# SciML/NeuralPDE.jl

Measured on NVIDIA H100. Metric: collocation-points/sec (loss+grad), higher is better.
Workload: dtype f32

## Files before the change

neuralpde.jl_b200/csrc/tc_common.cuh:

```cuda
#pragma once
#include <cuda_runtime.h>
#include <stdint.h>
#include "tc_types.h"
#include "ffma_kernel.cuh"
#include "tc_prims.cuh"
#include "tail.cuh"

namespace pinn {

constexpr int kNH = kTcThreads / 128;
static_assert(kTcThreads == 512, "the MMA chains are spread over four warpgroups");
constexpr int GW = 4;
constexpr int GWB = 2;

template <int N>
__device__ __forceinline__ float pick(const float* v, int idx) {
  float r = v[0];
#pragma unroll
  for (int i = 1; i < N; ++i) r = (idx == i) ? v[i] : r;
  return r;
}
template <int N>
__device__ __forceinline__ void add_at(float* v, int idx, float x) {
#pragma unroll
// ... 425 lines not shown
      const int n_params = P.n_params;
      for (int j = 0; j < n_params; ++j) {
        float v = warp_sum<float>(pbar[j] * g);
        if (lane == 0) atomicAdd(&partial[P.param_off + j], v);
      }
    }
  }
  __syncthreads();
}

struct DbgSpan {
  long long c0;
  unsigned long long g0;
};
__device__ __forceinline__ DbgSpan dbg_span_begin(const long long* dbg) {
  DbgSpan s{0, 0};
#ifdef PINN_DEBUG
  if (dbg && threadIdx.x == 0) {
    s.c0 = clock64();
    asm volatile("mov.u64 %0, %globaltimer;" : "=l"(s.g0));
  }
#endif
  return s;
}

template <typename CS>
__device__ __forceinline__ void cta_finish(const TcCommonArgs& a, const CS& cs, const DbgSpan& span, const Misc& ms,
                                           const DevProblem& P, bool want_grad) {
  extern __shared__ __align__(1024) uint8_t smem[];
  const int tid = threadIdx.x;
#ifdef PINN_DEBUG
  if (tid == 0 && cs.dbg) cs.dbg[999] = cs.dbg_n;
  if (a.dbg && tid == 0 && blockIdx.x < 250) {
    unsigned long long g1;
    unsigned int smid;
    asm volatile("mov.u64 %0, %globaltimer;" : "=l"(g1));
    asm volatile("mov.u32 %0, %smid;" : "=r"(smid));
    long long* rec = a.dbg + 1000 + 4 * blockIdx.x;
    rec[0] = (long long)span.g0; rec[1] = (long long)g1; rec[2] = clock64() - span.c0; rec[3] = smid;
  }
#endif
  if (tid < PINN_MAX_TERMS) a.term_sums[(long long)blockIdx.x * PINN_MAX_TERMS + tid] = ms.tsum[tid];
  if (a.tail.state)
    fused_tail<float, kTcThreads>(a.tail, a.partial, a.partial_stride, a.term_sums, P.n_theta, P.n_terms, want_grad ? 1 : 0,
                                  reinterpret_cast<float*>(smem + a.off_P));
}


template <int C, typename CS>
__device__ __forceinline__ void finish_forward(CS* cs, const DevTerm& tm, int slot, const Misc& ms, const float* bl, const Tid& t,
                                               const float (&u)[C]) {
  __syncthreads();
  dbg_mark(cs, 15);
#pragma unroll
  for (int c = 0; c < C; ++c) atomicAdd(&ms.scratch[c * kTcPts + t.p], u[c]);
  __syncthreads();
  if (t.hh == 0) {
    float s[C];
#pragma unroll
    for (int c = 0; c < C; ++c) s[c] = ms.scratch[c * kTcPts + t.p];
    s[0] += *bl;
    const int n_taps = tm.n_taps;
    for (int tt = 0; tt < n_taps; ++tt)
      if (tm.tap_slot[tt] == slot) {
        const int tch = tm.tap_ch[tt];
        float v = s[0];
#pragma unroll
        for (int c = 1; c < C; ++c) v = (tch == c) ? s[c] : v;
        ms.taps[tt * kTcPts + t.p] = v;
      }
  }
  __syncthreads();
  dbg_mark(cs, 16);
}

template <int C>
__device__ __forceinline__ void gather_ubar(const DevTerm& tm, int slot, const Misc& ms, int p, float (&ub)[C]) {
#pragma unroll
  for (int c = 0; c < C; ++c) ub[c] = 0.f;
  const int n_taps = tm.n_taps;
  for (int tt = 0; tt < n_taps; ++tt)
    if (tm.tap_slot[tt] == slot) {
      const float g = ms.tapbar[tt * kTcPts + p];
      const int tch = tm.tap_ch[tt];
#pragma unroll
      for (int c = 0; c < C; ++c) ub[c] += (tch == c) ? g : 0.f;
    }
}

template <int C>
__device__ __forceinline__ void last_layer_grad(const Tid& t, const float (&ub)[C], int nL, float* gw, float* gb, uint32_t u_tile,
                                                uint32_t h_tile, uint32_t h_stride, uint32_t h_lbo, uint32_t acol, int rows) {
  if (t.hh == 0) {
    const float s = warp_sum<float>(ub[0]);
    if (t.lane == 0) atomicAdd(gb, s);
    uint32_t w[8];
#pragma unroll
    for (int c = 0; c < 8; ++c) w[c] = 0u;
#pragma unroll
    for (int c = 0; c < C; ++c) {
      const uint32_t hi = tc::pack_bf16(ub[c], 0.f);
      w[c] = hi | (bf16x2_lo(ub[c], 0.f, hi) << 16);
    }
    sts_v4(u_tile + tc::swz_chunk(t.p, 0), w[0], w[1], w[2], w[3]);
    sts_v4(u_tile + tc::swz_chunk(t.p, 1), w[4], w[5], w[6], w[7]);
  }
  tc::fence_async_smem();
  __syncthreads();
  {
    const uint32_t idesc = tc::make_idesc(16, 1, 1);
    const uint64_t db = tc::make_desc(u_tile, 0, 1024);
#pragma unroll 1
    for (int c = 0; c < C; ++c)
      mma_chain(acol + 16 * c, tc::make_desc(h_tile + c * h_stride, h_lbo, 1024), db, 2048, 2048, kTcPts / 16, idesc, 0);
  }
  __syncthreads();
  if (t.hh == 0 && t.q * 32 < rows) {
    const int o = t.q * 32 + t.lane;
    float acc = 0.f;
#pragma unroll
    for (int c = 0; c < C; ++c) {
      float v[2];
      acc_ld2(t.lane_addr + acol + 16 * c + 2 * c, v);
      acc += v[0] + v[1];
    }
    if (o < nL) atomicAdd(gw + o, acc);
  }
  __syncthreads();
}

__device__ __forceinline__ void flush_wgrad(const Tid& t, uint32_t wcol, uint32_t bcol, int rows, int n_in, int n_out, float* gw,
                                            float* gb) {
  if (t.q * 32 < rows) {
    const int o = t.q * 32 + t.lane;
    if (t.hh == 0) {
      float v[2];
      acc_ld2(t.lane_addr + bcol, v);
      if (o < n_out) atomicAdd(gb + o, v[0]);
    }
    const int part = n_in / kNH;
#pragma unroll 1
    for (int k0 = t.hh * part; k0 < (t.hh + 1) * part; k0 += 4) {
      float v[4];
      acc_ld4(t.lane_addr + wcol + k0, v);
      if (o < n_out) {
#pragma unroll
        for (int i = 0; i < 4; ++i) atomicAdd(gw + o + (long long)n_out * (k0 + i), v[i]);
      }
    }
  }
}

template <int N1>
__device__ __forceinline__ void coord_tiles(const Tid& t, uint32_t b_tile, const float (&x)[PINN_MAX_IN],
                                            const int (&dir1)[N1 > 0 ? N1 : 1], bool x_lo) {
  if (t.tid >= kTcPts) return;
  uint32_t hi[4], lo[4];
#pragma unroll
  for (int k = 0; k < 4; ++k) {
    hi[k] = tc::pack_bf16(x[2 * k], x[2 * k + 1]);
    lo[k] = bf16x2_lo(x[2 * k], x[2 * k + 1], hi[k]);
  }
  const uint32_t c0a = b_tile + tc::swz_chunk(t.p, 0), c1a = b_tile + tc::swz_chunk(t.p, 1);
  sts_v4(c0a, hi[0], hi[1], hi[2], hi[3]);
  sts_v4(c1a, 0x00003f80u, 0u, 0u, 0u);
  if (x_lo) {
    sts_v4(c0a + (1 + N1) * kTileBytes, lo[0], lo[1], lo[2], lo[3]);
    sts_v4(c1a + (1 + N1) * kTileBytes, 0u, 0u, 0u, 0u);
  }
#pragma unroll
  for (int j = 0; j < N1; ++j) {
    const int d = dir1[j];
    uint32_t w[4];
#pragma unroll
    for (int k = 0; k < 4; ++k) w[k] = (d == 2 * k) ? 0x00003f80u : ((d == 2 * k + 1) ? 0x3f800000u : 0u);
    sts_v4(c0a + (1 + j) * kTileBytes, w[0], w[1], w[2], w[3]);
    sts_v4(c1a + (1 + j) * kTileBytes, 0u, 0u, 0u, 0u);
  }
}
template <int N1>
__device__ __forceinline__ void layer0_grad(const Tid& t, uint32_t z_tile, uint32_t z_stride, uint32_t z_lbo, uint32_t b_tile,
                                            bool x_lo, uint32_t acol, int rows, int n1w, int d_in, float* gw0, float* gb0) {
  tc::fence_async_smem();
  __syncthreads();
  {
    const uint32_t idesc = tc::make_idesc(16, 1, 1);
    const uint64_t a0 = tc::make_desc(z_tile, z_lbo, 1024);
    mma_chain(acol, a0, tc::make_desc(b_tile, 0, 1024), 2048, 2048, kTcPts / 16, idesc, 0);
    if (x_lo) mma_chain(acol, a0, tc::make_desc(b_tile + (1 + N1) * kTileBytes, 0, 1024), 2048, 2048, kTcPts / 16, idesc, 1);
#pragma unroll 1
    for (int j = 0; j < N1; ++j)
      mma_chain(acol, tc::make_desc(z_tile + (1 + j) * z_stride, z_lbo, 1024), tc::make_desc(b_tile + (1 + j) * kTileBytes, 0, 1024),
                2048, 2048, kTcPts / 16, idesc, 1);
  }
  __syncthreads();
  if (t.hh == 0 && t.q * 32 < rows) {
    const int o = t.q * 32 + t.lane;
    float v[16];
    tc::acc_ld16(t.lane_addr + acol, v);
    if (o < n1w) {
#pragma unroll
      for (int k = 0; k < PINN_MAX_IN; ++k)
        if (k < d_in) atomicAdd(gw0 + o + (long long)n1w * k, v[k]);
      atomicAdd(gb0 + o, v[8]);
    }
  }
}

#define PINN_TC_CASE(maxc, a1, a2, pu, CALL)                                                  \
  {                                                                                           \
    constexpr int A1 = a1, A2 = a2;                                                           \
    constexpr bool PU = pu;                                                                   \
    if constexpr (1 + A1 + A2 <= (maxc)) {                                                    \
      if (_ak == 1) { constexpr int AK = 1; CALL; } else { constexpr int AK = 0; CALL; }     \
    }                                                                                         \
  }                                                                                           \
  break
#define PINN_TC_DISPATCH(maxc, n1, n2, pure, ak, CALL)                                        \
  do {                                                                                        \
    const int _ak = (ak);                                                                     \
    const int _key = ((n1) * 8 + (n2)) * 2 + ((pure) ? 1 : 0);                                \
    switch (_key) {                                                                           \
      case (0 * 8 + 0) * 2: case (0 * 8 + 0) * 2 + 1: PINN_TC_CASE(maxc, 0, 0, true, CALL);   \
      case (1 * 8 + 0) * 2: case (1 * 8 + 0) * 2 + 1: PINN_TC_CASE(maxc, 1, 0, true, CALL);   \
      case (2 * 8 + 0) * 2: case (2 * 8 + 0) * 2 + 1: PINN_TC_CASE(maxc, 2, 0, true, CALL);   \
      case (3 * 8 + 0) * 2: case (3 * 8 + 0) * 2 + 1: PINN_TC_CASE(maxc, 3, 0, true, CALL);   \
      case (4 * 8 + 0) * 2: case (4 * 8 + 0) * 2 + 1: PINN_TC_CASE(maxc, 4, 0, true, CALL);   \
      case (1 * 8 + 1) * 2: case (1 * 8 + 1) * 2 + 1: PINN_TC_CASE(maxc, 1, 1, true, CALL);   \
      case (2 * 8 + 1) * 2 + 1: PINN_TC_CASE(maxc, 2, 1, true, CALL);                         \
      case (2 * 8 + 1) * 2: PINN_TC_CASE(maxc, 2, 1, false, CALL);                            \
      case (3 * 8 + 1) * 2 + 1: PINN_TC_CASE(maxc, 3, 1, true, CALL);                         \
      case (3 * 8 + 1) * 2: PINN_TC_CASE(maxc, 3, 1, false, CALL);                            \
      case (2 * 8 + 2) * 2 + 1: PINN_TC_CASE(maxc, 2, 2, true, CALL);                         \
      case (2 * 8 + 2) * 2: PINN_TC_CASE(maxc, 2, 2, false, CALL);                            \
      default: break;                                                                         \
    }                                                                                         \
  } while (0)

}
```

neuralpde.jl_b200/csrc/tc_kernel.cu:

```cuda
#include "tc_common.cuh"

namespace pinn {

using Fp = FpBlock<kTcW>;

struct CtaShared : CtaBase {
  int split, off_Q;
  uint8_t* stash;
  TcNetSmem nets[PINN_MAX_NETS];
};

struct LoopCtx {
  uint32_t fp;
  uint32_t bt;
  uint32_t tP;
  uint32_t tQ;
  float* gb;
  float* gw;
  uint32_t taddr;
  int act, split, p, lane, g0, g1, flag;
  __device__ __forceinline__ LoopCtx(uint32_t fp_, uint32_t bt_, uint32_t tP_, uint32_t tQ_, const Tid& t, int act_, int ng,
                                     int flag_, int split_ = 0, float* gb_ = nullptr, float* gw_ = nullptr)
      : fp(fp_), bt(bt_), tP(tP_), tQ(tQ_), gb(gb_), gw(gw_), taddr(t.lane_addr), act(act_), split(split_), p(t.p), lane(t.lane),
        g0(t.hh * (ng / kNH)), g1((t.hh + 1) * (ng / kNH)), flag(flag_) {}
};

template <int N1, int N2, bool PURE, int AK>
__device__ __forceinline__ void l0_fwd_loop(const LoopCtx lc, const PassInfo<N1, N2> pi, const float* xp, float* up) {
  constexpr int C = 1 + N1 + N2;
  float x[PINN_MAX_IN], u[C];
#pragma unroll
  for (int k = 0; k < PINN_MAX_IN; ++k) x[k] = xp[k];
#pragma unroll
  for (int c = 0; c < C; ++c) u[c] = up[c];
#pragma unroll 1
  for (int g = lc.g0; g < lc.g1; ++g) {
    float h[C][GW];
#pragma unroll
    for (int i = 0; i < GW; i += 2) {
      float za[C], zb2[C];
      first_layer_elem<kTcW>(lc.fp, pi, x, g * GW + i, za);
      first_layer_elem<kTcW>(lc.fp, pi, x, g * GW + i + 1, zb2);
      P2 zz[C], hv[C];
#pragma unroll
      for (int c = 0; c < C; ++c) zz[c] = mk2(za[c], zb2[c]);
      chain_fwd<N1, N2, PURE, AK, P2>(lc.act, pi.ch, zz, hv);
#pragma unroll
      for (int c = 0; c < C; ++c) { h[c][i] = hv[c].v.x; h[c][i + 1] = hv[c].v.y; }
      if (lc.flag) {
        const float w0 = lds_f32(lc.fp + (Fp::WL + g * GW + i) * 4), w1 = lds_f32(lc.fp + (Fp::WL + g * GW + i + 1) * 4);
#pragma unroll
        for (int c = 0; c < C; ++c) u[c] = fmaf(w1, hv[c].v.y, fmaf(w0, hv[c].v.x, u[c]));
      }
    }
#pragma unroll
    for (int c = 0; c < C; ++c) store_half(lc.tP + c * kTileBytes, lc.tQ + c * kTileBytes, lc.p, g * GW, h[c], lc.split != 0);
  }
#pragma unroll
  for (int c = 0; c < C; ++c) up[c] = u[c];
}

template <int C, int NK, bool SPLIT>
__device__ __forceinline__ void fwd_mma(float (&d)[C][16], uint32_t sP, uint32_t sQ, uint32_t whi, uint32_t wlo) {
  const int wg = threadIdx.x >> 7;
  const uint32_t aoff = (wg & 1) * 8192u, boff = (wg >> 1) * 32u * 128u;
  const uint64_t dwhi = tc::make_desc(whi + boff, 0, 1024), dwlo = tc::make_desc(wlo + boff, 0, 1024);
  tc::wgmma_fence();
#pragma unroll
  for (int c = 0; c < C; ++c) {
    const uint64_t dahi = tc::make_desc(sP + c * kTileBytes + aoff, 0, 1024);
    const uint64_t dalo = tc::make_desc(sQ + c * kTileBytes + aoff, 0, 1024);
#pragma unroll
    for (int pr = 0; pr < (SPLIT ? 3 : 1); ++pr) {
      const uint64_t a = (pr == 2) ? dalo : dahi, b = (pr == 1) ? dwlo : dwhi;
#pragma unroll
      for (int k = 0; k < NK; ++k)
        tc::wgmma_n32<0, 0>(d[c], a + 2 * k, b + 2 * k, (pr | k) ? 1u : 0u);
    }
  }
  tc::wgmma_commit();
  tc::wgmma_wait0();
}
template <int C>
__device__ __forceinline__ void fwd_mma_any(float (&d)[C][16], uint32_t sP, uint32_t sQ, uint32_t whi, uint32_t wlo, int nk,
                                            bool split) {
  switch (nk * 2 + (split ? 1 : 0)) {
    case 2: fwd_mma<C, 1, false>(d, sP, sQ, whi, wlo); break;
    case 3: fwd_mma<C, 1, true>(d, sP, sQ, whi, wlo); break;
    case 4: fwd_mma<C, 2, false>(d, sP, sQ, whi, wlo); break;
    case 5: fwd_mma<C, 2, true>(d, sP, sQ, whi, wlo); break;
    case 6: fwd_mma<C, 3, false>(d, sP, sQ, whi, wlo); break;
    case 7: fwd_mma<C, 3, true>(d, sP, sQ, whi, wlo); break;
    case 8: fwd_mma<C, 4, false>(d, sP, sQ, whi, wlo); break;
    default: fwd_mma<C, 4, true>(d, sP, sQ, whi, wlo); break;
  }
}

template <int N1, int N2, bool PURE, int AK, int C>
__device__ __forceinline__ void tl_fwd_frag(const float (&d)[C][16], const LoopCtx lc, const Chan<N1, N2> ch, float* scratch) {
  const int wg = threadIdx.x >> 7, w = (threadIdx.x >> 5) & 3;
  const int row0 = 64 * (wg & 1) + 16 * w + (lc.lane >> 2);
  const int col0 = 32 * (wg >> 1) + 2 * (lc.lane & 3);
  float u[2][C];
#pragma unroll
  for (int r = 0; r < 2; ++r)
#pragma unroll
    for (int c = 0; c < C; ++c) u[r][c] = 0.f;
#pragma unroll
  for (int i = 0; i < 16; i += 2) {
    const int rh = (i >> 1) & 1;
    const int row = row0 + 8 * rh, col = col0 + 8 * (i >> 2);
    P2 zz[C], hv[C];
    zz[0] = mk2(d[0][i] + lds_f32(lc.bt + col * 4), d[0][i + 1] + lds_f32(lc.bt + (col + 1) * 4));
#pragma unroll
    for (int c = 1; c < C; ++c) zz[c] = mk2(d[c][i], d[c][i + 1]);
    chain_fwd<N1, N2, PURE, AK, P2>(lc.act, ch, zz, hv);
    const uint32_t off = tc::swz_off(row, col);
#pragma unroll
    for (int c = 0; c < C; ++c) {
      const uint32_t hx = tc::pack_bf16(hv[c].v.x, hv[c].v.y);
      asm volatile("st.shared.b32 [%0], %1;" ::"r"(lc.tP + c * kTileBytes + off), "r"(hx) : "memory");
      if (lc.split)
        asm volatile("st.shared.b32 [%0], %1;" ::"r"(lc.tQ + c * kTileBytes + off), "r"(bf16x2_lo(hv[c].v.x, hv[c].v.y, hx))
                     : "memory");
    }
    if (lc.flag) {
      const float w0 = lds_f32(lc.fp + (Fp::WL + col) * 4), w1 = lds_f32(lc.fp + (Fp::WL + col + 1) * 4);
#pragma unroll
      for (int c = 0; c < C; ++c) u[rh][c] = fmaf(w1, hv[c].v.y, fmaf(w0, hv[c].v.x, u[rh][c]));
    }
  }
  if (lc.flag) {
#pragma unroll
    for (int r = 0; r < 2; ++r)
#pragma unroll
      for (int c = 0; c < C; ++c) {
        float s = u[r][c];
        s += __shfl_xor_sync(0xffffffffu, s, 1);
        s += __shfl_xor_sync(0xffffffffu, s, 2);
        if ((lc.lane & 3) == 0) atomicAdd(&scratch[c * kTcPts + row0 + 8 * r], s);
      }
  }
}

constexpr uint32_t kHalfBytes = kTileBytes / 2;

template <int C, int NK>
__device__ __forceinline__ void rec_mma(float (&d)[C][8], uint32_t sQ, uint32_t whi) {
  const uint64_t dw = tc::make_desc(whi + (threadIdx.x >> 7) * 16u * 128u, 0, 1024);
  tc::wgmma_fence();
#pragma unroll
  for (int c = 0; c < C; ++c) {
    const uint64_t da = tc::make_desc(sQ + c * kTileBytes, 0, 1024);
#pragma unroll
    for (int k = 0; k < NK; ++k) tc::wgmma_n16<0, 0>(d[c], da + 2 * k, dw + 2 * k, k ? 1u : 0u);
  }
  tc::wgmma_commit();
  tc::wgmma_wait0();
}
template <int C>
__device__ __forceinline__ void rec_mma_any(float (&d)[C][8], uint32_t sQ, uint32_t whi, int nk) {
  switch (nk) {
    case 1: rec_mma<C, 1>(d, sQ, whi); break;
    case 2: rec_mma<C, 2>(d, sQ, whi); break;
    case 3: rec_mma<C, 3>(d, sQ, whi); break;
    default: rec_mma<C, 4>(d, sQ, whi); break;
  }
}
template <int C, int NKO>
__device__ __forceinline__ void dgrad_mma(float (&d)[C][8], uint32_t sQ, uint32_t whi) {
  const uint32_t poff = kHalfBytes + (threadIdx.x >> 7) * 16u * 128u;
  const uint64_t dw = tc::make_desc(whi, 0, 1024);
  tc::wgmma_fence();
#pragma unroll
  for (int c = 0; c < C; ++c) {
    const uint64_t dz = tc::make_desc(sQ + c * kTileBytes + poff, 0, 1024);
#pragma unroll
    for (int k = 0; k < NKO; ++k)
      tc::wgmma_n16<1, 0>(d[c], dw + 128 * k, dz + 2 * k, k ? 1u : 0u);
  }
  tc::wgmma_commit();
  tc::wgmma_wait0();
}
template <int C>
__device__ __forceinline__ void dgrad_mma_any(float (&d)[C][8], uint32_t sQ, uint32_t whi, int nko) {
  switch (nko) {
    case 1: dgrad_mma<C, 1>(d, sQ, whi); break;
    case 2: dgrad_mma<C, 2>(d, sQ, whi); break;
    case 3: dgrad_mma<C, 3>(d, sQ, whi); break;
    default: dgrad_mma<C, 4>(d, sQ, whi); break;
  }
}
template <int C>
__device__ __forceinline__ void wgrad_mma(float (&dw)[32], float (&db)[8], uint32_t sQ, uint32_t s_ones) {
  const uint32_t poff = (threadIdx.x >> 7) * 16u * 128u;
  const uint64_t d1 = tc::make_desc(s_ones, 0, 0);
  tc::wgmma_fence();
#pragma unroll
  for (int c = 0; c < C; ++c) {
    const uint64_t dh = tc::make_desc(sQ + c * kTileBytes + poff, 0, 1024);
    const uint64_t dz = tc::make_desc(sQ + c * kTileBytes + kHalfBytes + poff, 0, 1024);
    tc::wgmma_n64<1, 1>(dw, dh, dz, c ? 1u : 0u);
  }
  tc::wgmma_n16<1, 1>(db, tc::make_desc(sQ + kHalfBytes + poff, 0, 1024), d1, 0u);
  tc::wgmma_commit();
  tc::wgmma_wait0();
}

__device__ __forceinline__ int hb_idx(int c, int k, int p) { return (c * 64 + k) * 64 + (p ^ ((((k >> 1) ^ k) & 3) << 3)); }

template <int C>
__device__ __forceinline__ void hbar_store(float* hbar, const float (&d)[C][8]) {
  const int wg = threadIdx.x >> 7, w = (threadIdx.x >> 5) & 3, lane = threadIdx.x & 31;
#pragma unroll
  for (int c = 0; c < C; ++c)
#pragma unroll
    for (int i = 0; i < 8; i += 2) {
      const int k = 16 * w + (lane >> 2) + 8 * ((i >> 1) & 1), p = 16 * wg + 8 * (i >> 2) + 2 * (lane & 3);
      *reinterpret_cast<float2*>(hbar + hb_idx(c, k, p)) = make_float2(d[c][i], d[c][i + 1]);
    }
}

template <int C>
__device__ __forceinline__ void hbar0_store(float* hand, const float (&d)[C][8], int h) {
  const int wg = threadIdx.x >> 7, w = (threadIdx.x >> 5) & 3, lane = threadIdx.x & 31;
#pragma unroll
  for (int c = 0; c < C; ++c)
#pragma unroll
    for (int i = 0; i < 8; i += 2) {
      const int k = 16 * w + (lane >> 2) + 8 * ((i >> 1) & 1), p = 64 * h + 16 * wg + 8 * (i >> 2) + 2 * (lane & 3);
      *reinterpret_cast<float2*>(hand + (c * 64 + k) * kAccRows + p) = make_float2(d[c][i], d[c][i + 1]);
    }
}

template <int NF>
__device__ __forceinline__ void frag_store_rows(float* base, int ld, const float (&d)[NF]) {
  const int w = (threadIdx.x >> 5) & 3, lane = threadIdx.x & 31;
  const bool odd = (lane & 1) != 0;
  float* row = base + (16 * w + (lane >> 2) + (odd ? 8 : 0)) * ld + 4 * ((lane >> 1) & 1);
#pragma unroll
  for (int j = 0; j < NF / 4; ++j) {
    const float r0 = __shfl_xor_sync(0xffffffffu, odd ? d[4 * j] : d[4 * j + 2], 1);
    const float r1 = __shfl_xor_sync(0xffffffffu, odd ? d[4 * j + 1] : d[4 * j + 3], 1);
    *reinterpret_cast<float4*>(row + 8 * j) =
        odd ? make_float4(r0, r1, d[4 * j + 2], d[4 * j + 3]) : make_float4(d[4 * j], d[4 * j + 1], r0, r1);
  }
}

template <int N1, int N2, bool PURE, int AK, int C>
__device__ __forceinline__ void tl_bwd_frag(const float (&d)[C][8], const LoopCtx lc, const Chan<N1, N2> ch, const float* ubs,
                                            const float* hbar, int h) {
  const int wg = threadIdx.x >> 7, w = (threadIdx.x >> 5) & 3;
  const int row0 = 16 * w + (lc.lane >> 2);
  const int col0 = 16 * wg + 2 * (lc.lane & 3);
#pragma unroll
  for (int i = 0; i < 8; i += 2) {
    const int row = row0 + 8 * ((i >> 1) & 1), col = col0 + 8 * (i >> 2);
    P2 zz[C], hv[C], zv[C];
    zz[0] = mk2(d[0][i] + lds_f32(lc.bt + col * 4), d[0][i + 1] + lds_f32(lc.bt + (col + 1) * 4));
#pragma unroll
    for (int c = 1; c < C; ++c) zz[c] = mk2(d[c][i], d[c][i + 1]);
    if (lc.flag) {
      const float w0 = lds_f32(lc.fp + (Fp::WL + col) * 4), w1 = lds_f32(lc.fp + (Fp::WL + col + 1) * 4);
#pragma unroll
      for (int c = 0; c < C; ++c) {
        const float u = ubs[c * kTcPts + 64 * h + row];
        hv[c] = mk2(w0 * u, w1 * u);
      }
    } else {
#pragma unroll
      for (int c = 0; c < C; ++c) hv[c] = mk2(hbar[hb_idx(c, col, row)], hbar[hb_idx(c, col + 1, row)]);
    }
    chain_bwd<N1, N2, PURE, AK, P2>(lc.act, ch, zz, hv, zv);
    const uint32_t off = kHalfBytes + tc::swz_off(row, col);
#pragma unroll
    for (int c = 0; c < C; ++c)
      asm volatile("st.shared.b32 [%0], %1;" ::"r"(lc.tQ + c * kTileBytes + off), "r"(tc::pack_bf16(zv[c].v.x, zv[c].v.y))
                   : "memory");
  }
}

template <int N1, int N2, bool PURE, int AK>
__device__ __forceinline__ void l0_bwd_store_loop(const LoopCtx lc, const PassInfo<N1, N2> pi, const float* xp) {
  constexpr int C = 1 + N1 + N2;
  float x[PINN_MAX_IN];
#pragma unroll
  for (int k = 0; k < PINN_MAX_IN; ++k) x[k] = xp[k];
#pragma unroll 1
  for (int g = lc.g0; g < lc.g1; ++g) {
    float hb[C][GWB];
#pragma unroll
    for (int c = 0; c < C; ++c) acc_ldg(lc.taddr + TM_X + c * 64 + g * GWB, hb[c]);
#pragma unroll
    for (int i = 0; i < GWB; i += 2) {
      float za[C], zb2[C];
      first_layer_elem<kTcW>(lc.fp, pi, x, g * GWB + i, za);
      first_layer_elem<kTcW>(lc.fp, pi, x, g * GWB + i + 1, zb2);
      P2 zz[C], hv[C], zv[C];
#pragma unroll
      for (int c = 0; c < C; ++c) { zz[c] = mk2(za[c], zb2[c]); hv[c] = mk2(hb[c][i], hb[c][i + 1]); }
      chain_bwd<N1, N2, PURE, AK, P2>(lc.act, pi.ch, zz, hv, zv);
#pragma unroll
      for (int c = 0; c <= N1; ++c) { hb[c][i] = zv[c].v.x; hb[c][i + 1] = zv[c].v.y; }
    }
#pragma unroll
    for (int c = 0; c <= N1; ++c) store_half(lc.tP + c * kTileBytes, lc.tP, lc.p, g * GWB, hb[c], false);
  }
}

template <int N1, int N2, bool PURE, int AK>
__device__ __forceinline__ void l0_bwd_loop(const LoopCtx lc, const PassInfo<N1, N2> pi, const float* xp, const float* ubp) {
  constexpr int C = 1 + N1 + N2;
  float x[PINN_MAX_IN], ub[C];
#pragma unroll
  for (int k = 0; k < PINN_MAX_IN; ++k) x[k] = xp[k];
#pragma unroll
  for (int c = 0; c < C; ++c) ub[c] = ubp[c];
  const int re = reduceg_elem(lc.lane);
  const bool rlead = reduceg_lead(lc.lane);
  const int n1w = pi.n1w;
#pragma unroll 1
  for (int g = lc.g0; g < lc.g1; ++g) {
    float hb[C][GW];
#pragma unroll
    for (int i = 0; i < GW; ++i) {
      const float wl = lds_f32(lc.fp + (Fp::WL + g * GW + i) * 4);
#pragma unroll
      for (int c = 0; c < C; ++c) hb[c][i] = wl * ub[c];
    }
    float zv0[GW], zvd[N1 > 0 ? N1 : 1][GW];
#pragma unroll
    for (int i = 0; i < GW; ++i) {
      float zz[C], hv[C], zv[C];
      first_layer_elem<kTcW>(lc.fp, pi, x, g * GW + i, zz);
#pragma unroll
      for (int c = 0; c < C; ++c) hv[c] = hb[c][i];
      chain_bwd<N1, N2, PURE, AK, float>(lc.act, pi.ch, zz, hv, zv);
      zv0[i] = zv[0];
#pragma unroll
      for (int jd = 0; jd < N1; ++jd) zvd[jd][i] = zv[1 + jd];
    }
    const float bs = warp_reduceg(zv0, lc.lane);
    if (rlead) atomicAdd(lc.gb + g * GW + re, bs);
#pragma unroll
    for (int k = 0; k < PINN_MAX_IN; ++k) {
      if (k < pi.d_in) {
        float gk[GW];
#pragma unroll
        for (int i = 0; i < GW; ++i) {
          float gg = zv0[i] * x[k];
#pragma unroll
          for (int jd = 0; jd < N1; ++jd) gg += (pi.dir1[jd] == k) ? zvd[jd][i] : 0.f;
          gk[i] = gg;
        }
        const float gs = warp_reduceg(gk, lc.lane);
        if (rlead) atomicAdd(lc.gw + g * GW + re + (long long)n1w * k, gs);
      }
    }
  }
}

template <int N1, int N2, bool PURE, int AK>
__device__ __noinline__ uint32_t net_forward(CtaShared* cs, const DevProblem* Pp, const DevTerm* tmp, int slot,
                                             int want_grad, uint32_t phase) {
  extern __shared__ __align__(1024) uint8_t smem[];
  constexpr int C = 1 + N1 + N2;
  const DevTerm& tm = *tmp;
  const int net_id = tm.used_net[slot];
  const DevNet& net = Pp->nets[net_id];
  const DevChan& dc = tm.chan[slot];
  const TcNetSmem ns = cs->nets[net_id];
  const float* fp = reinterpret_cast<const float*>(smem + ns.fp);
  uint8_t* tP = smem + cs->off_P;
  uint8_t* tQ = smem + cs->off_Q;
  const Misc ms = misc_of(smem + cs->off_misc, cs->mx_dim, cs->mx_taps);
  const uint32_t accm = 0;
  const bool split = cs->split != 0;
  PassInfo<N1, N2> pi;
  load_pass<N1, N2>(pi, net, dc);
  const int TL = pi.TL;
  const Tid t = tid_of();
  const int tid = t.tid, p = t.p;
  float x[PINN_MAX_IN];
#pragma unroll
  for (int k = 0; k < PINN_MAX_IN; ++k) x[k] = (k < pi.d_in) ? ms.Xs[dc.rows[k] * kTcPts + p] : 0.f;
  uint8_t* stash_slot = cs->stash + (size_t)slot * cs->tl_max * kTcMaxC * kTileBytes;

  dbg_mark(cs, 10);
  float u[C];
#pragma unroll
  for (int c = 0; c < C; ++c) u[c] = 0.f;
  if (tid < C * kTcPts / 4) reinterpret_cast<float4*>(ms.scratch)[tid] = make_float4(0.f, 0.f, 0.f, 0.f);
  {
    const LoopCtx lc(tc::smem_u32(fp), tc::smem_u32(fp), tc::smem_u32(tP), tc::smem_u32(tQ), t, net.acts[0], pi.n1w / GW, TL == 0, split);
    l0_fwd_loop<N1, N2, PURE, AK>(lc, pi, x, u);
  }
  for (int l = 1; l <= TL; ++l) {
    const int n_in = net.dims[l], n_out = net.dims[l + 1];
    const int act = net.acts[l];
    tc::fence_async_smem();
    __syncthreads();
    dbg_mark(cs, 11);
    if (want_grad && tid == 0) {
      for (int c = 0; c < C; ++c)
        tc::bulk_store(stash_slot + (size_t)(l - 1) * kTcMaxC * kTileBytes + (size_t)c * kTileBytes, tP + c * kTileBytes, kTileBytes);
      tc::bulk_commit();
    }
    float d[C][16];
    {
      const uint32_t sP = tc::smem_u32(tP), sQ = tc::smem_u32(tQ);
      const uint32_t whi = tc::smem_u32(smem + ns.w_hi[l - 1]), wlo = tc::smem_u32(smem + ns.w_lo[l - 1]);
      const int nk = n_in / 16;
      fwd_mma_any<C>(d, sP, sQ, whi, wlo, nk, split);
    }
    dbg_mark(cs, 13);
    if (want_grad && tid == 0) tc::bulk_wait_read0();
    __syncthreads();
    dbg_mark(cs, 14);
    const LoopCtx lc(tc::smem_u32(fp), tc::smem_u32(fp) + (Fp::BT + (l - 1) * 64) * 4, tc::smem_u32(tP), tc::smem_u32(tQ), t, act, 0, l == TL, split);
    tl_fwd_frag<N1, N2, PURE, AK, C>(d, lc, pi.ch, ms.scratch);
  }
  finish_forward<C>(cs, tm, slot, ms, fp + Fp::BL, t, u);
  return phase;
}

template <int N1, int N2, bool PURE, int AK>
__device__ __noinline__ uint32_t net_backward(CtaShared* cs, const DevProblem* Pp, const DevTerm* tmp, int slot,
                                              uint32_t phase) {
  extern __shared__ __align__(1024) uint8_t smem[];
  constexpr int C = 1 + N1 + N2;
  const DevTerm& tm = *tmp;
  const int net_id = tm.used_net[slot];
  const DevNet& net = Pp->nets[net_id];
  const DevChan& dc = tm.chan[slot];
  const TcNetSmem ns = cs->nets[net_id];
  const float* fp = reinterpret_cast<const float*>(smem + ns.fp);
  uint8_t* tP = smem + cs->off_P;
  uint8_t* tQ = smem + cs->off_Q;
  const Misc ms = misc_of(smem + cs->off_misc, cs->mx_dim, cs->mx_taps);
  const uint32_t accm = 0;
  float* partial = cs->partial;
  PassInfo<N1, N2> pi;
  load_pass<N1, N2>(pi, net, dc);
  const int L = pi.L, TL = pi.TL;
  const Tid t = tid_of();
  const int tid = t.tid, p = t.p;
  uint32_t ld_phase = (phase >> 1) & 1u;
  float x[PINN_MAX_IN];
#pragma unroll
  for (int k = 0; k < PINN_MAX_IN; ++k) x[k] = (k < pi.d_in) ? ms.Xs[dc.rows[k] * kTcPts + p] : 0.f;
  uint8_t* stash_slot = cs->stash + (size_t)slot * cs->tl_max * kTcMaxC * kTileBytes;

  dbg_mark(cs, 20);
  float ub[C];
  gather_ubar<C>(tm, slot, ms, p, ub);
  if (t.hh == 0) {
#pragma unroll
    for (int c = 0; c < C; ++c) ms.scratch[c * kTcPts + p] = ub[c];
  }
  last_layer_grad<C>(t, ub, pi.nL, partial + net.w_off[L - 1], partial + net.b_off[L - 1], tc::smem_u32(tQ), tc::smem_u32(tP),
                     kTileBytes, 0u, accm + TM_Y, kTcW);

  const uint32_t sP = tc::smem_u32(tP), sQ = tc::smem_u32(tQ);
  const int act0 = net.acts[0];
  float* gb0 = partial + net.b_off[0];
  float* gw0 = partial + net.w_off[0];
  if (TL == 0) {
    __syncthreads();
    dbg_mark(cs, 29);
    const LoopCtx lc(tc::smem_u32(fp), tc::smem_u32(fp), sP, sQ, t, act0, pi.n1w / GW, 1, 0, gb0, gw0);
    l0_bwd_loop<N1, N2, PURE, AK>(lc, pi, x, ub);
  }

  const int wg = tid >> 7;
  float* hbar = reinterpret_cast<float*>(tP);
  float* wpart = reinterpret_cast<float*>(tP);
  float* bpart = reinterpret_cast<float*>(tQ + kHalfBytes);
  float* hand = tc::s_acc + TM_X * kAccRows;
#pragma unroll 1
  for (int h = 0; h < (TL > 0 ? 2 : 0); ++h) {
    for (int l = TL; l >= 1; --l) {
      const int n_in = net.dims[l], n_out = net.dims[l + 1];
      const int act = net.acts[l];
      float* gb = partial + net.b_off[l];
      float* gw = partial + net.w_off[l];
      const float* bt = fp + Fp::BT + (l - 1) * 64;
      const uint32_t whi = tc::smem_u32(smem + ns.w_hi[l - 1]);
      dbg_mark(cs, 21);
      if (tid == 0 && l == TL) {
        const uint8_t* src = stash_slot + (size_t)(l - 1) * kTcMaxC * kTileBytes + h * kHalfBytes;
        tc::mbar_arrive_expect_tx(ms.bar_ld, C * kHalfBytes);
        for (int c = 0; c < C; ++c) tc::bulk_load(tQ + c * kTileBytes, src + (size_t)c * kTileBytes, kHalfBytes, ms.bar_ld);
      }
      wait_bar(ms.bar_ld, ld_phase);
      dbg_mark(cs, 22);
      {
        float d[C][8];
        rec_mma_any<C>(d, sQ, whi, n_in / 16);
        __syncthreads();
        dbg_mark(cs, 24);
        const LoopCtx lc(tc::smem_u32(fp), tc::smem_u32(bt), sP, sQ, t, act, 0, l == TL);
        tl_bwd_frag<N1, N2, PURE, AK, C>(d, lc, pi.ch, ms.scratch, hbar, h);
      }
      tc::fence_async_smem();
      __syncthreads();
      dbg_mark(cs, 26);
      float db0, db2;
      {
        float dw[32], db[8];
        wgrad_mma<C>(dw, db, sQ, tc::smem_u32(smem + cs->off_ones));
        frag_store_rows(wpart + wg * 64 * 64, 64, dw);
        db0 = db[0]; db2 = db[2];
      }
      float d[C][8];
      dgrad_mma_any<C>(d, sQ, whi, n_out / 16);
      __syncthreads();
      dbg_mark(cs, 27);
      if (tid == 0 && l > 1) {
        const uint8_t* src = stash_slot + (size_t)(l - 2) * kTcMaxC * kTileBytes + h * kHalfBytes;
        tc::mbar_arrive_expect_tx(ms.bar_ld, C * kHalfBytes);
        for (int c = 0; c < C; ++c) tc::bulk_load(tQ + c * kTileBytes, src + (size_t)c * kTileBytes, kHalfBytes, ms.bar_ld);
      }
      if ((t.lane & 3) == 0) {
        const int o = 16 * (t.warp & 3) + (t.lane >> 2);
        bpart[wg * 64 + o] = db0;
        bpart[wg * 64 + o + 8] = db2;
      }
      __syncthreads();
      dbg_mark(cs, 28);
      if ((reinterpret_cast<uintptr_t>(gw) & 15) == 0) {
        const float4* wp4 = reinterpret_cast<const float4*>(wpart);
#pragma unroll 1
        for (int e = tid; e < 64 * 16; e += kTcThreads) {
          const int k = e >> 4, o = (e & 15) * 4;
          if (k < n_in && o < n_out) {
            const float4 a = wp4[e], b = wp4[1024 + e], c = wp4[2048 + e], q = wp4[3072 + e];
            float4* g = reinterpret_cast<float4*>(gw + o + (long long)n_out * k);
            float4 v = *g;
            v.x += ((a.x + b.x) + c.x) + q.x;
            v.y += ((a.y + b.y) + c.y) + q.y;
            v.z += ((a.z + b.z) + c.z) + q.z;
            v.w += ((a.w + b.w) + c.w) + q.w;
            *g = v;
          }
        }
      } else {
#pragma unroll 1
        for (int e = tid; e < 64 * 64; e += kTcThreads) {
          const int k = e >> 6, o = e & 63;
          if (k < n_in && o < n_out) gw[o + (long long)n_out * k] += ((wpart[e] + wpart[4096 + e]) + wpart[8192 + e]) + wpart[12288 + e];
        }
      }
      if (tid < n_out) gb[tid] += ((bpart[tid] + bpart[64 + tid]) + bpart[128 + tid]) + bpart[192 + tid];
      __syncthreads();
      if (l > 1) hbar_store<C>(hbar, d);
      else hbar0_store<C>(hand, d, h);
    }
  }
  if (TL > 0) {
    __syncthreads();
    dbg_mark(cs, 29);
    coord_tiles<N1>(t, sQ, x, pi.dir1, N2 > 0);
    const LoopCtx lc(tc::smem_u32(fp), tc::smem_u32(fp), sP, sQ, t, act0, pi.n1w / GWB, 0);
    l0_bwd_store_loop<N1, N2, PURE, AK>(lc, pi, x);
    layer0_grad<N1>(t, sP, kTileBytes, 0u, sQ, N2 > 0, accm + TM_Y, kTcW, pi.n1w, pi.d_in, gw0, gb0);
  }

  __syncthreads();
  dbg_mark(cs, 30);
  return (ld_phase << 1) | (phase & 1u);
}


__global__ void __launch_bounds__(kTcThreads, 1) tc_loss_grad_kernel(const __grid_constant__ TcArgs args) {
  extern __shared__ __align__(1024) uint8_t smem[];
  __shared__ CtaShared cs;
  const int tid = threadIdx.x;
  const DevProblem* Pp = args.prob;
  const DevProblem& P = *Pp;
  const Misc ms = misc_of(smem + args.off_misc, args.mx_dim, args.mx_taps);
  float* partial = args.partial + (long long)blockIdx.x * args.partial_stride;
  const bool want_grad = (args.mode == 0);
  const float* theta = args.theta;
  const DbgSpan span = dbg_span_begin(args.dbg);

  for (long long i = (long long)tid * 32; i < args.n_theta; i += (long long)kTcThreads * 32) tc::prefetch_l2(theta + i);
  {
    const char* nets0 = reinterpret_cast<const char*>(&Pp->nets[0]);
    const char* terms0 = reinterpret_cast<const char*>(&Pp->terms[0]);
    const int nb_nets = args.n_nets * (int)sizeof(DevNet), nb_terms = args.n_terms * (int)sizeof(DevTerm);
    if (tid == 0) tc::prefetch_l2(Pp);
    for (int o = tid * 128; o < nb_nets; o += kTcThreads * 128) tc::prefetch_l2(nets0 + o);
    for (int o = tid * 128; o < nb_terms; o += kTcThreads * 128) tc::prefetch_l2(terms0 + o);
    const int tile = args.tile_begin + (int)blockIdx.x;
    if (tile < args.tile_end && tid < 32) {
      int ti = 0;
      while (ti + 1 < args.n_terms && tile >= args.dyn[ti + 1].tile0) ++ti;
      const long long p0 = (long long)(tile - args.dyn[ti].tile0) * kTcPts;
      const long long row_bytes = 4ll * args.term_dim[ti];
      const long long off = p0 * row_bytes + (long long)tid * 128;
      if (off < args.dyn[ti].n * row_bytes) tc::prefetch_l2(reinterpret_cast<const char*>(args.dyn[ti].pts) + off);
    }
  }
  if (tid == 0) {
    tc::mbar_init(ms.bar_ld, 1);
    tc::fence_barrier_init();
    cs.split = args.split; cs.off_Q = args.off_Q;
    cs.stash = args.stash + (long long)blockIdx.x * args.stash_per_cta;
    for (int k = 0; k < PINN_MAX_NETS; ++k) cs.nets[k] = args.nets[k];
    cta_base_init(cs, args, partial);
  }
  if (tid == 0) tc::s_acc = args.acc + (size_t)blockIdx.x * kAccCols * kAccRows;
  cta_setup(args, ms, partial, P.n_theta, want_grad);
  for (int kn = 0; kn < P.n_nets; ++kn) {
    const DevNet& net = P.nets[kn];
    const TcNetSmem& ns = args.nets[kn];
    if (ns.fp < 0) continue;
    stage_fp_block<kTcW>(reinterpret_cast<float*>(smem + ns.fp), net, theta);
    const int L = net.n_layers;
    {
      constexpr int kItMax = kTcMaxTL * 512 / kTcThreads;
      const int n_items = (L - 2) * 512;
      float w[kItMax][8];
#pragma unroll
      for (int it = 0; it < kItMax; ++it) {
        const int i = tid + it * kTcThreads;
        if (i < n_items) {
          const int l = 1 + i / 512, r = i & 511;
          const int o = r & 63, kc = r >> 6;
          const int n_in = net.dims[l], n_out = net.dims[l + 1];
          const long long woff = net.w_off[l];
#pragma unroll
          for (int e = 0; e < 8; ++e) {
            const int k = kc * 8 + e;
            w[it][e] = (o < n_out && k < n_in) ? __ldg(&theta[woff + o + (long long)n_out * k]) : 0.f;
          }
        }
      }
#pragma unroll
      for (int it = 0; it < kItMax; ++it) {
        const int i = tid + it * kTcThreads;
        if (i < n_items) {
          const int l = 1 + i / 512, r = i & 511;
          const int o = r & 63, kc = r >> 6;
          uint8_t* thi = smem + ns.w_hi[l - 1];
          uint8_t* tlo = smem + ns.w_lo[l - 1];
          const float* v = w[it];
          uint32_t h[4];
#pragma unroll
          for (int e = 0; e < 4; ++e) h[e] = tc::pack_bf16(v[2 * e], v[2 * e + 1]);
          *reinterpret_cast<uint4*>(thi + tc::swz_chunk(o, kc)) = make_uint4(h[0], h[1], h[2], h[3]);
          if (args.split)
            *reinterpret_cast<uint4*>(tlo + tc::swz_chunk(o, kc)) = make_uint4(
                bf16x2_lo(v[0], v[1], h[0]), bf16x2_lo(v[2], v[3], h[1]), bf16x2_lo(v[4], v[5], h[2]), bf16x2_lo(v[6], v[7], h[3]));
        }
      }
    }
  }
  tc::fence_async_smem();
  __syncthreads();
  dbg_mark(&cs, 2);
  uint32_t phase = 0;

  for (int tile = args.tile_begin + blockIdx.x; tile < args.tile_end; tile += gridDim.x) {
    if (tid >= 128 && tid < 128 + (int)((sizeof(DevNet) * PINN_MAX_NETS + 127) / 128))
      tc::prefetch_l1(reinterpret_cast<const char*>(&P.nets[0]) + (tid - 128) * 128);
    uint32_t ldp = (phase >> 1) & 1u;
    const TileRef tr = stage_tile(args, P, ms, tile, ldp);
    phase = (phase & 1u) | (ldp << 1);
    const DevTerm* tmp = &P.terms[tr.ti];
    const DevTerm& tm = *tmp;
    const int n_used = tm.n_used;
    dbg_mark(&cs, 3);

    for (int slot = 0; slot < n_used; ++slot) {
      const int k1 = tm.chan[slot].n1, k2 = tm.chan[slot].n2, pu = tm.chan[slot].pure;
      const int ak = args.net_ak[tm.used_net[slot]];
      PINN_TC_DISPATCH(kTcMaxC, k1, k2, pu, ak, (phase = net_forward<A1, A2, PU, AK>(&cs, Pp, tmp, slot, want_grad ? 1 : 0, phase)));
    }

    dbg_mark(&cs, 4);
    residual_step(args, P, tm, ms, tr, smem + args.off_Q, (size_t)args.off_Q_bytes, partial, want_grad);

    dbg_mark(&cs, 5);
    if (want_grad) {
      if (tid == 0) tc::bulk_wait0();
      __syncthreads();
      dbg_mark(&cs, 6);
      for (int slot = n_used - 1; slot >= 0; --slot) {
        const int k1 = tm.chan[slot].n1, k2 = tm.chan[slot].n2, pu = tm.chan[slot].pure;
        const int ak = args.net_ak[tm.used_net[slot]];
        if (n_used > 1) {
          PINN_TC_DISPATCH(kTcMaxC, k1, k2, pu, ak, (phase = net_forward<A1, A2, PU, AK>(&cs, Pp, tmp, slot, 0, phase)));
        }
        PINN_TC_DISPATCH(kTcMaxC, k1, k2, pu, ak, (phase = net_backward<A1, A2, PU, AK>(&cs, Pp, tmp, slot, phase)));
      }
    }
  }

  __syncthreads();
  dbg_mark(&cs, 7);
  cta_finish(args, cs, span, ms, P, want_grad);
}

size_t tc_misc_bytes(int mx_dim, int mx_taps) {
  return (size_t)mx_dim * kTcPts * 4 + 2 * (size_t)mx_taps * kTcPts * 4 + (size_t)kTcMaxC * kTcPts * 4 + kTcPts * 4 +
         PINN_MAX_TERMS * 8 + 16 + 16;
}

cudaError_t tc_launch(const TcArgs& a, int grid, size_t smem, cudaStream_t st) {
  return launch_fused_kernel<tc_loss_grad_kernel>(a, grid, kTcThreads, smem, st);
}

}
```

Before: 98.58 million.

## Fold layer-0 backward into each half-pass using smem hbar and wgmma

Layer-0 backward now runs inside each of the two half-passes (l0_half). It reads hbar straight from shared memory instead of staging it through the tensor-memory/accumulator region (hbar0_store plus acc_ldg), and computes the layer-0 weight gradient with a per-warpgroup wgmma reduction rather than the separate full-tile mma_chain in layer0_grad. This removes the accumulator round-trip and the extra full-width pass over 128 points, trading them for more syncthreads per half, a noinline call, and a four-way partial sum in shared memory.

Result: faster. 108.9 million, median of 6 (+10.5%).

```diff
diff --git a/neuralpde.jl_b200/csrc/tc_common.cuh b/neuralpde.jl_b200/csrc/tc_common.cuh
--- a/neuralpde.jl_b200/csrc/tc_common.cuh
+++ b/neuralpde.jl_b200/csrc/tc_common.cuh
@@ -601,16 +601,15 @@
 }
 
 template <int N1>
-__device__ __forceinline__ void coord_tiles(const Tid& t, uint32_t b_tile, const float (&x)[PINN_MAX_IN],
-                                            const int (&dir1)[N1 > 0 ? N1 : 1], bool x_lo) {
-  if (t.tid >= kTcPts) return;
+__device__ __forceinline__ void coord_row(uint32_t b_tile, int row, const float (&x)[PINN_MAX_IN],
+                                          const int (&dir1)[N1 > 0 ? N1 : 1], bool x_lo) {
   uint32_t hi[4], lo[4];
 #pragma unroll
   for (int k = 0; k < 4; ++k) {
     hi[k] = tc::pack_bf16(x[2 * k], x[2 * k + 1]);
     lo[k] = bf16x2_lo(x[2 * k], x[2 * k + 1], hi[k]);
   }
-  const uint32_t c0a = b_tile + tc::swz_chunk(t.p, 0), c1a = b_tile + tc::swz_chunk(t.p, 1);
+  const uint32_t c0a = b_tile + tc::swz_chunk(row, 0), c1a = b_tile + tc::swz_chunk(row, 1);
   sts_v4(c0a, hi[0], hi[1], hi[2], hi[3]);
   sts_v4(c1a, 0x00003f80u, 0u, 0u, 0u);
   if (x_lo) {
@@ -626,6 +625,12 @@
     sts_v4(c0a + (1 + j) * kTileBytes, w[0], w[1], w[2], w[3]);
     sts_v4(c1a + (1 + j) * kTileBytes, 0u, 0u, 0u, 0u);
   }
+}
+template <int N1>
+__device__ __forceinline__ void coord_tiles(const Tid& t, uint32_t b_tile, const float (&x)[PINN_MAX_IN],
+                                            const int (&dir1)[N1 > 0 ? N1 : 1], bool x_lo) {
+  if (t.tid >= kTcPts) return;
+  coord_row<N1>(b_tile, t.p, x, dir1, x_lo);
 }
 template <int N1>
 __device__ __forceinline__ void layer0_grad(const Tid& t, uint32_t z_tile, uint32_t z_stride, uint32_t z_lbo, uint32_t b_tile,
diff --git a/neuralpde.jl_b200/csrc/tc_kernel.cu b/neuralpde.jl_b200/csrc/tc_kernel.cu
--- a/neuralpde.jl_b200/csrc/tc_kernel.cu
+++ b/neuralpde.jl_b200/csrc/tc_kernel.cu
@@ -17,11 +17,10 @@
   uint32_t tQ;
   float* gb;
   float* gw;
-  uint32_t taddr;
   int act, split, p, lane, g0, g1, flag;
   __device__ __forceinline__ LoopCtx(uint32_t fp_, uint32_t bt_, uint32_t tP_, uint32_t tQ_, const Tid& t, int act_, int ng,
                                      int flag_, int split_ = 0, float* gb_ = nullptr, float* gw_ = nullptr)
-      : fp(fp_), bt(bt_), tP(tP_), tQ(tQ_), gb(gb_), gw(gw_), taddr(t.lane_addr), act(act_), split(split_), p(t.p), lane(t.lane),
+      : fp(fp_), bt(bt_), tP(tP_), tQ(tQ_), gb(gb_), gw(gw_), act(act_), split(split_), p(t.p), lane(t.lane),
         g0(t.hh * (ng / kNH)), g1((t.hh + 1) * (ng / kNH)), flag(flag_) {}
 };
 
@@ -207,6 +206,21 @@
   tc::wgmma_wait0();
 }
 
+template <int N1, int N2>
+__device__ __forceinline__ void l0_mma(float (&d)[8], uint32_t sQ) {
+  const uint32_t poff = (threadIdx.x >> 7) * 16u * 128u;
+  const uint64_t dz0 = tc::make_desc(sQ + kHalfBytes + poff, 0, 1024);
+  tc::wgmma_fence();
+  tc::wgmma_n16<1, 1>(d, dz0, tc::make_desc(sQ + poff, 0, 1024), 0u);
+  if (N2 > 0) tc::wgmma_n16<1, 1>(d, dz0, tc::make_desc(sQ + (1 + N1) * kTileBytes + poff, 0, 1024), 1u);
+#pragma unroll
+  for (int j = 0; j < N1; ++j)
+    tc::wgmma_n16<1, 1>(d, tc::make_desc(sQ + (1 + j) * kTileBytes + kHalfBytes + poff, 0, 1024),
+                        tc::make_desc(sQ + (1 + j) * kTileBytes + poff, 0, 1024), 1u);
+  tc::wgmma_commit();
+  tc::wgmma_wait0();
+}
+
 __device__ __forceinline__ int hb_idx(int c, int k, int p) { return (c * 64 + k) * 64 + (p ^ ((((k >> 1) ^ k) & 3) << 3)); }
 
 template <int C>
@@ -218,18 +232,6 @@
     for (int i = 0; i < 8; i += 2) {
       const int k = 16 * w + (lane >> 2) + 8 * ((i >> 1) & 1), p = 16 * wg + 8 * (i >> 2) + 2 * (lane & 3);
       *reinterpret_cast<float2*>(hbar + hb_idx(c, k, p)) = make_float2(d[c][i], d[c][i + 1]);
-    }
-}
-
-template <int C>
-__device__ __forceinline__ void hbar0_store(float* hand, const float (&d)[C][8], int h) {
-  const int wg = threadIdx.x >> 7, w = (threadIdx.x >> 5) & 3, lane = threadIdx.x & 31;
-#pragma unroll
-  for (int c = 0; c < C; ++c)
-#pragma unroll
-    for (int i = 0; i < 8; i += 2) {
-      const int k = 16 * w + (lane >> 2) + 8 * ((i >> 1) & 1), p = 64 * h + 16 * wg + 8 * (i >> 2) + 2 * (lane & 3);
-      *reinterpret_cast<float2*>(hand + (c * 64 + k) * kAccRows + p) = make_float2(d[c][i], d[c][i + 1]);
     }
 }
 
@@ -281,16 +283,16 @@
 }
 
 template <int N1, int N2, bool PURE, int AK>
-__device__ __forceinline__ void l0_bwd_store_loop(const LoopCtx lc, const PassInfo<N1, N2> pi, const float* xp) {
+__device__ __forceinline__ void l0_bwd_store_loop(const LoopCtx lc, const PassInfo<N1, N2> pi, const float (&x)[PINN_MAX_IN],
+                                                  const float* hbar) {
   constexpr int C = 1 + N1 + N2;
-  float x[PINN_MAX_IN];
-#pragma unroll
-  for (int k = 0; k < PINN_MAX_IN; ++k) x[k] = xp[k];
 #pragma unroll 1
   for (int g = lc.g0; g < lc.g1; ++g) {
     float hb[C][GWB];
 #pragma unroll
-    for (int c = 0; c < C; ++c) acc_ldg(lc.taddr + TM_X + c * 64 + g * GWB, hb[c]);
+    for (int c = 0; c < C; ++c)
+#pragma unroll
+      for (int i = 0; i < GWB; ++i) hb[c][i] = hbar[hb_idx(c, g * GWB + i, lc.p)];
 #pragma unroll
     for (int i = 0; i < GWB; i += 2) {
       float za[C], zb2[C];
@@ -304,7 +306,7 @@
       for (int c = 0; c <= N1; ++c) { hb[c][i] = zv[c].v.x; hb[c][i + 1] = zv[c].v.y; }
     }
 #pragma unroll
-    for (int c = 0; c <= N1; ++c) store_half(lc.tP + c * kTileBytes, lc.tP, lc.p, g * GWB, hb[c], false);
+    for (int c = 0; c <= N1; ++c) store_half(lc.tQ + c * kTileBytes + kHalfBytes, lc.tQ, lc.p, g * GWB, hb[c], false);
   }
 }
 
@@ -356,6 +358,46 @@
         const float gs = warp_reduceg(gk, lc.lane);
         if (rlead) atomicAdd(lc.gw + g * GW + re + (long long)n1w * k, gs);
       }
+    }
+  }
+}
+
+template <int N1, int N2, bool PURE, int AK>
+__device__ __noinline__ void l0_half(uint32_t fpa, uint8_t* tP, uint8_t* tQ, int act0, const PassInfo<N1, N2> pi, const float* xs,
+                                     const int* rows, int h, float* gw0, float* gb0) {
+  const Tid t = tid_of();
+  const int tid = t.tid, wg = tid >> 7;
+  const uint32_t sP = tc::smem_u32(tP), sQ = tc::smem_u32(tQ);
+  const float* hbar = reinterpret_cast<const float*>(tP);
+  float* lpart = reinterpret_cast<float*>(tP);
+  {
+    const int pl = 32 * (t.warp & 1) + t.lane, ng = pi.n1w / (8 * GWB);
+    float x[PINN_MAX_IN];
+#pragma unroll
+    for (int k = 0; k < PINN_MAX_IN; ++k) x[k] = (k < pi.d_in) ? xs[rows[k] * kTcPts + 64 * h + pl] : 0.f;
+    if (tid < 64) coord_row<N1>(sQ, pl, x, pi.dir1, N2 > 0);
+    __syncthreads();
+    LoopCtx lc(fpa, fpa, sP, sQ, t, act0, 0, 0);
+    lc.p = pl;
+    lc.g0 = (t.warp >> 1) * ng;
+    lc.g1 = lc.g0 + ng;
+    l0_bwd_store_loop<N1, N2, PURE, AK>(lc, pi, x, hbar);
+  }
+  tc::fence_async_smem();
+  __syncthreads();
+  {
+    float d[8];
+    l0_mma<N1, N2>(d, sQ);
+    frag_store_rows(lpart + wg * 64 * 16, 16, d);
+  }
+  __syncthreads();
+  const int n1w = pi.n1w, d_in = pi.d_in;
+#pragma unroll 1
+  for (int e = tid; e < 64 * 16; e += kTcThreads) {
+    const int o = e >> 4, k = e & 15;
+    if (o < n1w && (k < d_in || k == 8)) {
+      float* g = (k == 8) ? gb0 + o : gw0 + o + (long long)n1w * k;
+      *g += ((lpart[e] + lpart[1024 + e]) + lpart[2048 + e]) + lpart[3072 + e];
     }
   }
 }
@@ -374,7 +416,6 @@
   uint8_t* tP = smem + cs->off_P;
   uint8_t* tQ = smem + cs->off_Q;
   const Misc ms = misc_of(smem + cs->off_misc, cs->mx_dim, cs->mx_taps);
-  const uint32_t accm = 0;
   const bool split = cs->split != 0;
   PassInfo<N1, N2> pi;
   load_pass<N1, N2>(pi, net, dc);
@@ -438,18 +479,15 @@
   uint8_t* tP = smem + cs->off_P;
   uint8_t* tQ = smem + cs->off_Q;
   const Misc ms = misc_of(smem + cs->off_misc, cs->mx_dim, cs->mx_taps);
-  const uint32_t accm = 0;
   float* partial = cs->partial;
   PassInfo<N1, N2> pi;
   load_pass<N1, N2>(pi, net, dc);
   const int L = pi.L, TL = pi.TL;
   const Tid t = tid_of();
-  const int tid = t.tid, p = t.p;
+  const int tid = t.tid, p = t.p, wg = tid >> 7;
   uint32_t ld_phase = (phase >> 1) & 1u;
-  float x[PINN_MAX_IN];
-#pragma unroll
-  for (int k = 0; k < PINN_MAX_IN; ++k) x[k] = (k < pi.d_in) ? ms.Xs[dc.rows[k] * kTcPts + p] : 0.f;
   uint8_t* stash_slot = cs->stash + (size_t)slot * cs->tl_max * kTcMaxC * kTileBytes;
+  const uint32_t sP = tc::smem_u32(tP), sQ = tc::smem_u32(tQ);
 
   dbg_mark(cs, 20);
   float ub[C];
@@ -458,25 +496,24 @@
 #pragma unroll
     for (int c = 0; c < C; ++c) ms.scratch[c * kTcPts + p] = ub[c];
   }
-  last_layer_grad<C>(t, ub, pi.nL, partial + net.w_off[L - 1], partial + net.b_off[L - 1], tc::smem_u32(tQ), tc::smem_u32(tP),
-                     kTileBytes, 0u, accm + TM_Y, kTcW);
-
-  const uint32_t sP = tc::smem_u32(tP), sQ = tc::smem_u32(tQ);
+  last_layer_grad<C>(t, ub, pi.nL, partial + net.w_off[L - 1], partial + net.b_off[L - 1], sQ, sP, kTileBytes, 0u, TM_Y, kTcW);
+
   const int act0 = net.acts[0];
   float* gb0 = partial + net.b_off[0];
   float* gw0 = partial + net.w_off[0];
   if (TL == 0) {
     __syncthreads();
     dbg_mark(cs, 29);
+    float x[PINN_MAX_IN];
+#pragma unroll
+    for (int k = 0; k < PINN_MAX_IN; ++k) x[k] = (k < pi.d_in) ? ms.Xs[dc.rows[k] * kTcPts + p] : 0.f;
     const LoopCtx lc(tc::smem_u32(fp), tc::smem_u32(fp), sP, sQ, t, act0, pi.n1w / GW, 1, 0, gb0, gw0);
     l0_bwd_loop<N1, N2, PURE, AK>(lc, pi, x, ub);
   }
 
-  const int wg = tid >> 7;
   float* hbar = reinterpret_cast<float*>(tP);
   float* wpart = reinterpret_cast<float*>(tP);
   float* bpart = reinterpret_cast<float*>(tQ + kHalfBytes);
-  float* hand = tc::s_acc + TM_X * kAccRows;
 #pragma unroll 1
   for (int h = 0; h < (TL > 0 ? 2 : 0); ++h) {
     for (int l = TL; l >= 1; --l) {
@@ -553,17 +590,10 @@
       }
       if (tid < n_out) gb[tid] += ((bpart[tid] + bpart[64 + tid]) + bpart[128 + tid]) + bpart[192 + tid];
       __syncthreads();
-      if (l > 1) hbar_store<C>(hbar, d);
-      else hbar0_store<C>(hand, d, h);
-    }
-  }
-  if (TL > 0) {
-    __syncthreads();
+      hbar_store<C>(hbar, d);
+    }
     dbg_mark(cs, 29);
-    coord_tiles<N1>(t, sQ, x, pi.dir1, N2 > 0);
-    const LoopCtx lc(tc::smem_u32(fp), tc::smem_u32(fp), sP, sQ, t, act0, pi.n1w / GWB, 0);
-    l0_bwd_store_loop<N1, N2, PURE, AK>(lc, pi, x);
-    layer0_grad<N1>(t, sP, kTileBytes, 0u, sQ, N2 > 0, accm + TM_Y, kTcW, pi.n1w, pi.d_in, gw0, gb0);
+    l0_half<N1, N2, PURE, AK>(tc::smem_u32(fp), tP, tQ, act0, pi, ms.Xs, dc.rows, h, gw0, gb0);
   }
 
   __syncthreads();
```
